# MeryylleA/Lunaris-Orion

Hardware: AMD Instinct MI355X
Metric: 128x128 sprites/sec, VAE training step (train_hybrid.py _process_batch), latent_dim=512 (higher is better)
Workload: dtype f16; 1 GPU; VAE-only training step (fwd+MSE/KL+bwd+clip+AdamW), per-GPU batch 64, latent_dim 512, teacher scalar 0 (--reward_scale 0 --quality_weight 0; the full hybrid step of BASELINE config 3 is the config3_full_hybrid object of a --full run at N=1), gradient_accumulation_steps 1, fp16 MFMA operands / fp32 accumulate, fp32 master weights; global_batch=64, latent_dim=512, parallelism=single, linear_weight_gradients=factored (never materialised)

## Files before the change

lunaris_orion_amd/csrc/lo_wgrad2.hip:

```cpp
#include "lo_conv.h"
#include "lo_conv_dev.h"

struct Wgrad2Args {
  const f16* a;
  const f16* f;
  float* slab;
  int B, Hc, Wc, Ca, Cf;
  int nsplit, chunks_per_split, nchunks;
  int packed_elems;
  int Cin;
  int wofs[4];
};

template <bool CONVT>
__global__ __launch_bounds__(512) void lo_wgrad_s2_mt(Wgrad2Args a) {
  constexpr int R = CONVT ? 4 : 3, NTAP = R * R;
  constexpr int TH = 4, TW = 8;
  constexpr int PH = 2 * TH + R - 1, PWH = 10;
  constexpr int PROWS = PH * 2 * PWH;
  constexpr int PQ = (PROWS + 7) / 8;
  static_assert(4 + PQ <= 32, "eight waves x four instructions per chunk");
  constexpr int A_BYTES = 32 * 128, P_BYTES = PQ * 1024;
  constexpr int STAGE = A_BYTES + P_BYTES;
  constexpr int NSTAGE = 3, D = 2;
  constexpr int NTW = (NTAP + 1) / 2;
  __shared__ __attribute__((aligned(1024))) unsigned char smem[NSTAGE * STAGE + 1024];

  const int tid = threadIdx.x, lane = tid & 63;
  const int wave = __builtin_amdgcn_readfirstlane(tid >> 6);
  const int wa = wave & 1, wf = (wave >> 1) & 1, wt = wave >> 2;
  const int tiles_f = (a.Cf + 63) >> 6, tiles = (a.Ca >> 6) * tiles_f;
  const int wid = lo_xcd_remap(blockIdx.x, gridDim.x);
  const int tile = wid % tiles, split = wid / tiles;
  const int a0 = (tile / tiles_f) * 64, f0 = (tile % tiles_f) * 64;
  const int q_begin = split * a.chunks_per_split;
  const int q_end = min(a.nchunks, q_begin + a.chunks_per_split);
  const int nq = q_end - q_begin;
  const int chunks_x = a.Wc / TW, chunks_img = chunks_x * (a.Hc / TH);
  const int Hf = 2 * a.Hc, Wf = 2 * a.Wc;
  const f16* zpage = reinterpret_cast<const f16*>(lo_zero_page);

  int s_kind[4], s_off[4], s_py[4], s_px[4];
  unsigned int s_lds[4];
#pragma unroll
  for (int j = 0; j < 4; ++j) {
    const int q = wave * 4 + j;
    const int row8 = lane >> 3, pos = lane & 7;
    if (q < 4) {
      const int arow = q * 8 + row8;
      s_kind[j] = 0;
      s_py[j] = arow / TW; s_px[j] = arow % TW;
      s_off[j] = (s_py[j] * a.Wc + s_px[j]) * a.Ca + a0 + ((((pos >> 1) ^ lo_tr_swz<128>(arow)) << 1) | (pos & 1)) * 8;
      s_lds[j] = (unsigned int)(q * 1024);
    } else if (q - 4 < PQ) {
      const int prow = (q - 4) * 8 + row8;
      const int py = prow / (2 * PWH), rem = prow - py * (2 * PWH), par = rem / PWH, hx = rem - par * PWH;
      const int px = 2 * hx + par;
      const int ch = f0 + ((((pos >> 1) ^ lo_tr_swz<128>(prow)) << 1) | (pos & 1)) * 8;
      const bool ok = prow < PROWS && px < 2 * TW + R - 1 && ch < a.Cf;
      s_kind[j] = ok ? 1 : 2;
      s_py[j] = py - 1; s_px[j] = px - 1;
      s_off[j] = ((py - 1) * Wf + (px - 1)) * a.Cf + ch;
      s_lds[j] = (unsigned int)(A_BYTES + (q - 4) * 1024);
    } else {
      s_kind[j] = 2; s_py[j] = s_px[j] = 0; s_off[j] = 0;
      s_lds[j] = (unsigned int)(NSTAGE * STAGE);
    }
  }
  int nx_q = q_begin;
  int nx_n = nx_q / chunks_img, nx_y, nx_x;
  {
    const int r = nx_q - nx_n * chunks_img;
    nx_y = (r / chunks_x) * TH;
    nx_x = (r % chunks_x) * TW;
  }
  const unsigned int smem_base = (unsigned int)(size_t)smem;
  auto issue = [&](int stage) __attribute__((always_inline)) {
    const bool live = nx_q < q_end;
    const int y0 = nx_y, x0 = nx_x;
    const size_t abase = ((size_t)(nx_n * a.Hc + y0) * a.Wc + x0) * a.Ca;
    const size_t fbase = ((size_t)(nx_n * Hf + 2 * y0) * Wf + 2 * x0) * a.Cf;
#pragma unroll
    for (int j = 0; j < 4; ++j) {
      const f16* src = zpage;
      if (live && s_kind[j] == 0) src = a.a + abase + s_off[j];
      if (live && s_kind[j] == 1) {
        const int fy = 2 * y0 + s_py[j], fx = 2 * x0 + s_px[j];
        if ((unsigned)fy < (unsigned)Hf && (unsigned)fx < (unsigned)Wf) src = a.f + (ptrdiff_t)fbase + s_off[j];
      }
      const unsigned int dst = s_lds[j] >= (unsigned int)(NSTAGE * STAGE) ? smem_base + s_lds[j] : smem_base + stage * STAGE + s_lds[j];
      lo_dma16(src, dst);
    }
    ++nx_q;
    nx_x += TW;
    if (nx_x >= a.Wc) { nx_x = 0; nx_y += TH; if (nx_y >= a.Hc) { nx_y = 0; ++nx_n; } }
  };

  const int q16 = lane >> 4, i16 = lane & 15;
  const int trow = 4 * q16 + (i16 >> 2);
  const int tsub = (i16 & 3) * 8;
  int aoff[2][2];
#pragma unroll
  for (int mi = 0; mi < 2; ++mi)
#pragma unroll
    for (int h = 0; h < 2; ++h) {
      const int Rr = trow + 16 * h, blk = wa * 2 + mi;
      aoff[mi][h] = Rr * 128 + ((blk ^ lo_tr_swz<128>(Rr)) * 32) + tsub;
    }
  int boff[NTW][2];
#pragma unroll
  for (int tt = 0; tt < NTW; ++tt)
#pragma unroll
    for (int h = 0; h < 2; ++h) {
      const int t = wt * NTW + tt;
      const int tq = t < NTAP ? t : 0;
      const int r = tq / R, s = tq % R;
      const int kk = trow + 16 * h, ky = kk / TW, kx = kk % TW;
      const int prow = ((2 * ky + r) * 2 + (s & 1)) * PWH + kx + (s >> 1);
      boff[tt][h] = A_BYTES + prow * 128 + (((wf * 2) ^ lo_tr_swz<128>(prow)) * 32) + tsub;
    }

  f32x4 acc[NTW][2][2];
#pragma unroll
  for (int tt = 0; tt < NTW; ++tt)
#pragma unroll
    for (int mi = 0; mi < 2; ++mi)
#pragma unroll
      for (int ni = 0; ni < 2; ++ni) acc[tt][mi][ni] = (f32x4){0.f, 0.f, 0.f, 0.f};

  auto tr = [&](const unsigned char* p) __attribute__((always_inline)) {
    return __builtin_amdgcn_ds_read_tr16_b64_v4f16((h16x4 __attribute__((address_space(3)))*)p);
  };
  auto frag = [&](const unsigned char* lo_p, const unsigned char* hi_p) __attribute__((always_inline)) {
    h16x4 lo = tr(lo_p), hi = tr(hi_p);
    return (f16x8){(f16)lo[0], (f16)lo[1], (f16)lo[2], (f16)lo[3], (f16)hi[0], (f16)hi[1], (f16)hi[2], (f16)hi[3]};
  };
  const bool f_live = f0 + wf * 32 < a.Cf;

  if (nq > 0) {
#pragma unroll
    for (int s = 0; s < D; ++s) issue(s);
    int rs = 0, ws = D % NSTAGE;
    for (int it = 0; it < nq; ++it) {
      LO_VMCNT(4 * (D - 1));
      __builtin_amdgcn_s_barrier();
      issue(ws);
      if (f_live) {
        const unsigned char* sbase = smem + rs * STAGE;
        f16x8 af[2];
#pragma unroll
        for (int mi = 0; mi < 2; ++mi) af[mi] = frag(sbase + aoff[mi][0], sbase + aoff[mi][1]);
#pragma unroll
        for (int tt = 0; tt < NTW; ++tt) {
          if (NTAP % 2 == 0 || tt + 1 < NTW || wt == 0) {
            f16x8 bf[2];
#pragma unroll
            for (int ni = 0; ni < 2; ++ni) bf[ni] = frag(sbase + (boff[tt][0] ^ (ni * 32)), sbase + (boff[tt][1] ^ (ni * 32)));
#pragma unroll
            for (int mi = 0; mi < 2; ++mi)
#pragma unroll
              for (int ni = 0; ni < 2; ++ni)
                acc[tt][mi][ni] = __builtin_amdgcn_mfma_f32_16x16x32_f16(af[mi], bf[ni], acc[tt][mi][ni], 0, 0, 0);
          }
        }
      }
      rs = (rs + 1 == NSTAGE) ? 0 : rs + 1;
      ws = (ws + 1 == NSTAGE) ? 0 : ws + 1;
    }
    LO_VMCNT(0);
  }
  if (!f_live) return;
  float* slab = a.slab + (size_t)split * a.packed_elems;
#pragma unroll
  for (int tt = 0; tt < NTW; ++tt) {
    const int t = wt * NTW + tt;
    if (t >= NTAP) continue;
    const int r = t / R, s = t % R;
#pragma unroll
    for (int mi = 0; mi < 2; ++mi)
#pragma unroll
      for (int ni = 0; ni < 2; ++ni) {
        const int cf = f0 + wf * 32 + ni * 16 + (lane & 15);
#pragma unroll
        for (int j = 0; j < 4; ++j) {
          const int ca = a0 + wa * 32 + mi * 16 + (lane >> 4) * 4 + j;
          size_t idx;
          if (CONVT) {
            const int p = ((r & 1) ? 0 : 2) + ((s & 1) ? 0 : 1), tp = (r >> 1) * 2 + (s >> 1);
            idx = (size_t)a.wofs[p] + (size_t)cf * (4 * a.Cin) + tp * a.Cin + ca;
          } else {
            idx = (size_t)ca * (9 * a.Cin) + t * a.Cin + cf;
          }
          if (cf < a.Cf) slab[idx] = acc[tt][mi][ni][j];
        }
      }
  }
}

int lo_wgrad2_run(const LoGeom& g, const LoWgradChoice& p, const f16* x, const f16* dy, float* slab, hipStream_t st) {
  LO_REQUIRE(p.kernel == LO_WK_WGRAD2, "lo_wgrad2_run: the plan names another weight-gradient kernel");
  const bool s2 = !p.convt;
  Wgrad2Args a;
  a.a = s2 ? dy : x; a.f = s2 ? x : dy; a.slab = slab;
  a.B = g.B; a.Hc = s2 ? g.Hout : g.Hin; a.Wc = s2 ? g.Wout : g.Win;
  a.Ca = s2 ? g.Cout : g.Cin; a.Cf = s2 ? g.Cin : g.Cout;
  a.nchunks = p.units; a.nsplit = p.nsplit; a.chunks_per_split = p.units_per_split;
  a.packed_elems = lo_geom_packed_elems(g);
  a.Cin = g.Cin;
  for (int q = 0; q < 4; ++q) a.wofs[q] = q < g.n_phase ? g.wofs[q] : 0;
  if (s2) hipLaunchKernelGGL((lo_wgrad_s2_mt<false>), p.grid, p.block, 0, st, a);
  else hipLaunchKernelGGL((lo_wgrad_s2_mt<true>), p.grid, p.block, 0, st, a);
  LO_LAUNCH_CHECK("wgrad_s2_mt");
  return LO_OK;
}
```

lunaris_orion_amd/csrc/lo_wgrad3.hip:

```cpp
#include "lo_conv.h"
#include "lo_conv_dev.h"

struct Wgrad3Args {
  const f16* x;
  const f16* dy;
  float* slab;
  int B, H, W, Cin, Cout;
  int nsplit, chunks_per_split, nchunks;
  int packed_elems;
#ifdef LO_STAMPS
  unsigned long long* stamps;
#endif
};
#ifdef LO_STAMPS
unsigned long long* g_lo_wgrad3_stamps = nullptr;
#define LO_T() __builtin_amdgcn_s_memtime()
#endif

template <int TH, int TW>
__global__ __launch_bounds__(512) void lo_wgrad3x3_mt(Wgrad3Args a) {
  static_assert(TH * TW == 32 && TW % 8 == 0, "a chunk is one 32-pixel K step");
  constexpr int PWP = TW + 2, PROWS = (TH + 2) * PWP;
  constexpr int PQ = (PROWS + 7) / 8;
  constexpr int PJ = (PQ + 3) / 4;
  constexpr int A_BYTES = 32 * 128;
  constexpr int P_BYTES = PQ * 1024;
  constexpr int STAGE = A_BYTES + P_BYTES;
  constexpr int NSTAGE = 4, D = 3;
  constexpr int XCHG_BYTES = 4 * 144 * 64 * 4;
  constexpr int LDS_BYTES = 2 * NSTAGE * STAGE > XCHG_BYTES ? 2 * NSTAGE * STAGE : XCHG_BYTES;
  __shared__ __attribute__((aligned(1024))) unsigned char smem_all[LDS_BYTES];

  const int tid = threadIdx.x, lane = tid & 63;
  const int wave8 = __builtin_amdgcn_readfirstlane(tid >> 6);
  const int grp = wave8 >> 2, wave = wave8 & 3;
  unsigned char* const smem = smem_all + grp * (NSTAGE * STAGE);
  const int wco = wave & 1, wci = wave >> 1;
  const int tiles_ci = a.Cin >> 6, tiles = (a.Cout >> 6) * tiles_ci;
  const int wid = lo_xcd_remap(blockIdx.x, gridDim.x);
  const int tile = wid % tiles, split = wid / tiles;
  const int co0 = (tile / tiles_ci) * 64, ci0 = (tile % tiles_ci) * 64;
  const int q_begin = split * a.chunks_per_split;
  const int q_end = min(a.nchunks, q_begin + a.chunks_per_split);
  const int nq = q_end - q_begin;
  const int chunks_x = a.W / TW, chunks_img = chunks_x * (a.H / TH);
  const f16* zpage = reinterpret_cast<const f16*>(lo_zero_page);

  const int drow = wave * 8 + (lane >> 3), dpos = lane & 7;
  const int d_ty = drow / TW, d_tx = drow % TW;
  const int d_lane = (d_ty * a.W + d_tx) * a.Cout + co0 + ((((dpos >> 1) ^ lo_tr_swz<128>(drow)) << 1) | (dpos & 1)) * 8;
  int p_py[PJ], p_px[PJ], p_lane[PJ];
#pragma unroll
  for (int j = 0; j < PJ; ++j) {
    const int prow = (j * 4 + wave) * 8 + (lane >> 3), pos = lane & 7;
    const int py = prow / PWP, px = prow - py * PWP;
    p_py[j] = prow < PROWS ? py - 1 : -100000;
    p_px[j] = px - 1;
    p_lane[j] = ((py - 1) * a.W + (px - 1)) * a.Cin + ci0 + ((((pos >> 1) ^ lo_tr_swz<128>(prow)) << 1) | (pos & 1)) * 8;
  }
  int nx_q = q_begin + grp;
  int nx_n = nx_q / chunks_img, nx_y, nx_x;
  {
    const int r = nx_q - nx_n * chunks_img;
    nx_y = (r / chunks_x) * TH;
    nx_x = (r % chunks_x) * TW;
  }
  auto issue = [&](int stage) __attribute__((always_inline)) {
    unsigned char* sa = smem + stage * STAGE;
    unsigned char* sp = sa + A_BYTES;
    const bool live = nx_q < q_end;
    const int y0 = nx_y, x0 = nx_x;
    const int pix0 = (nx_n * a.H + y0) * a.W + x0;
    {
      const f16* src = live ? a.dy + ((size_t)pix0 * a.Cout + d_lane) : zpage;
      lo_dma16(src, (unsigned int)(size_t)(sa + wave * 1024));
    }
#pragma unroll
    for (int j = 0; j < PJ; ++j) {
      if (j * 4 + wave < PQ) {
        const bool ok = live && (unsigned)(y0 + p_py[j]) < (unsigned)a.H && (unsigned)(x0 + p_px[j]) < (unsigned)a.W;
        const f16* src = ok ? a.x + ((size_t)pix0 * a.Cin + p_lane[j]) : zpage;
        lo_dma16(src, (unsigned int)(size_t)(sp + (j * 4 + wave) * 1024));
      }
    }
    nx_q += 2;
    nx_x += 2 * TW;
    if (nx_x >= a.W) {
      nx_x -= a.W; nx_y += TH;
      if (nx_x >= a.W) { nx_x -= a.W; nx_y += TH; }
      if (nx_y >= a.H) { nx_y -= a.H; ++nx_n; if (nx_y >= a.H) { nx_y -= a.H; ++nx_n; } }
    }
  };
  int lpt = 1;
#pragma unroll
  for (int j = 0; j < PJ; ++j) lpt += (j * 4 + wave < PQ) ? 1 : 0;

  const int q16 = lane >> 4, i16 = lane & 15;
  const int trow = 4 * q16 + (i16 >> 2);
  const int tsub = (i16 & 3) * 8;
  int aoff[2][2];
#pragma unroll
  for (int mi = 0; mi < 2; ++mi)
#pragma unroll
    for (int h = 0; h < 2; ++h) {
      const int R = trow + 16 * h, blk = wco * 2 + mi;
      aoff[mi][h] = R * 128 + ((blk ^ lo_tr_swz<128>(R)) * 32) + tsub;
    }
  int boff[9][2];
#pragma unroll
  for (int t = 0; t < 9; ++t)
#pragma unroll
    for (int h = 0; h < 2; ++h) {
      const int kk = trow + 16 * h;
      const int R = (kk / TW + t / 3) * PWP + kk % TW + t % 3;
      boff[t][h] = A_BYTES + R * 128 + (((wci * 2) ^ lo_tr_swz<128>(R)) * 32) + tsub;
    }

  f32x4 acc[9][2][2];
#pragma unroll
  for (int t = 0; t < 9; ++t)
#pragma unroll
    for (int mi = 0; mi < 2; ++mi)
#pragma unroll
      for (int ni = 0; ni < 2; ++ni) acc[t][mi][ni] = (f32x4){0.f, 0.f, 0.f, 0.f};

  auto tr = [&](const unsigned char* p) __attribute__((always_inline)) {
    return __builtin_amdgcn_ds_read_tr16_b64_v4f16((h16x4 __attribute__((address_space(3)))*)p);
  };
  auto frag = [&](const unsigned char* lo_p, const unsigned char* hi_p) __attribute__((always_inline)) {
    h16x4 lo = tr(lo_p), hi = tr(hi_p);
    return (f16x8){(f16)lo[0], (f16)lo[1], (f16)lo[2], (f16)lo[3], (f16)hi[0], (f16)hi[1], (f16)hi[2], (f16)hi[3]};
  };

  const int nit = (nq + 1) >> 1;
  auto compute = [&](int rs) __attribute__((always_inline)) {
    const unsigned char* sbase = smem + rs * STAGE;
    f16x8 af[2], bf[2][3][2];
#pragma unroll
    for (int mi = 0; mi < 2; ++mi) af[mi] = frag(sbase + aoff[mi][0], sbase + aoff[mi][1]);
#pragma unroll
    for (int tt = 0; tt < 3; ++tt)
#pragma unroll
      for (int ni = 0; ni < 2; ++ni) bf[0][tt][ni] = frag(sbase + (boff[tt][0] ^ (ni * 32)), sbase + (boff[tt][1] ^ (ni * 32)));
#pragma unroll
    for (int gq = 0; gq < 3; ++gq) {
      if (gq < 2) {
#pragma unroll
        for (int tt = 0; tt < 3; ++tt)
#pragma unroll
          for (int ni = 0; ni < 2; ++ni)
            bf[(gq + 1) & 1][tt][ni] = frag(sbase + (boff[3 * gq + 3 + tt][0] ^ (ni * 32)), sbase + (boff[3 * gq + 3 + tt][1] ^ (ni * 32)));
      }
#pragma unroll
      for (int tt = 0; tt < 3; ++tt)
#pragma unroll
        for (int mi = 0; mi < 2; ++mi)
#pragma unroll
          for (int ni = 0; ni < 2; ++ni)
            acc[3 * gq + tt][mi][ni] = __builtin_amdgcn_mfma_f32_16x16x32_f16(af[mi], bf[gq & 1][tt][ni], acc[3 * gq + tt][mi][ni], 0, 0, 0);
    }
  };
#ifdef LO_STAMPS
  const unsigned long long t_start = LO_T();
  unsigned long long t_loop = t_start, acc_w = 0, acc_i = 0, acc_c = 0;
#endif
  if (nit > 0) {
#pragma unroll
    for (int s = 0; s < D; ++s) issue(s);
#ifdef LO_STAMPS
    t_loop = LO_T();
#endif
    int rs = 0, ws = D % NSTAGE;
    for (int it = 0; it < nit; ++it) {
#ifdef LO_STAMPS
      const unsigned long long ta = LO_T();
#endif
      if (lpt == 4) LO_VMCNT(8); else if (lpt == 3) LO_VMCNT(6); else LO_VMCNT(4);
      __builtin_amdgcn_s_barrier();
#ifdef LO_STAMPS
      const unsigned long long tb = LO_T();
#endif
      if (grp == 0) issue(ws);
#ifdef LO_STAMPS
      const unsigned long long tc = LO_T();
#endif
      compute(rs);
#ifdef LO_STAMPS
      asm volatile("s_nop 0" ::: "memory");
      const unsigned long long td = LO_T();
#endif
      if (grp == 1) issue(ws);
#ifdef LO_STAMPS
      const unsigned long long te = LO_T();
      acc_w += tb - ta; acc_i += (tc - tb) + (te - td); acc_c += td - tc;
#endif
      rs = (rs + 1 == NSTAGE) ? 0 : rs + 1;
      ws = (ws + 1 == NSTAGE) ? 0 : ws + 1;
    }
    LO_VMCNT(0);
  }
#ifdef LO_STAMPS
  const unsigned long long t_loop_end = LO_T();
#endif
  __syncthreads();
  float* xch = reinterpret_cast<float*>(smem_all) + (size_t)wave * 144 * 64 + lane;
  if (grp == 1) {
#pragma unroll
    for (int t = 0; t < 9; ++t)
#pragma unroll
      for (int mi = 0; mi < 2; ++mi)
#pragma unroll
        for (int ni = 0; ni < 2; ++ni)
#pragma unroll
          for (int j = 0; j < 4; ++j) xch[(((t * 2 + mi) * 2 + ni) * 4 + j) * 64] = acc[t][mi][ni][j];
  }
  __syncthreads();
#ifdef LO_STAMPS
  if (a.stamps && lane == 0) {
    unsigned long long* d = a.stamps + ((size_t)blockIdx.x * 8 + wave8) * 16;
    d[0] = t_start; d[1] = t_loop; d[2] = t_loop_end; d[3] = LO_T(); d[4] = acc_w; d[5] = acc_i; d[6] = acc_c;
  }
#endif
  if (grp == 1) return;
#pragma unroll
  for (int t = 0; t < 9; ++t)
#pragma unroll
    for (int mi = 0; mi < 2; ++mi)
#pragma unroll
      for (int ni = 0; ni < 2; ++ni)
#pragma unroll
        for (int j = 0; j < 4; ++j) acc[t][mi][ni][j] += xch[(((t * 2 + mi) * 2 + ni) * 4 + j) * 64];
  float* slab = a.slab + (size_t)split * a.packed_elems;
  const int Ktot = 9 * a.Cin;
#pragma unroll
  for (int t = 0; t < 9; ++t)
#pragma unroll
    for (int mi = 0; mi < 2; ++mi)
#pragma unroll
      for (int ni = 0; ni < 2; ++ni) {
        const int c = ci0 + wci * 32 + ni * 16 + (lane & 15);
#pragma unroll
        for (int j = 0; j < 4; ++j) {
          const int n = co0 + wco * 32 + mi * 16 + (lane >> 4) * 4 + j;
          slab[(size_t)n * Ktot + t * a.Cin + c] = acc[t][mi][ni][j];
        }
      }
#ifdef LO_STAMPS
  if (a.stamps && lane == 0) a.stamps[((size_t)blockIdx.x * 8 + wave8) * 16 + 7] = LO_T();
#endif
}

int lo_wgrad3_run(const LoGeom& g, const LoWgradChoice& p, const f16* x, const f16* dy, float* slab, hipStream_t st) {
  LO_REQUIRE(p.kernel == LO_WK_WGRAD3, "lo_wgrad3_run: the plan names another weight-gradient kernel");
  Wgrad3Args a;
  a.x = x; a.dy = dy; a.slab = slab;
  a.B = g.B; a.H = g.Hin; a.W = g.Win; a.Cin = g.Cin; a.Cout = g.Cout;
  a.nchunks = p.units; a.nsplit = p.nsplit; a.chunks_per_split = p.units_per_split;
  a.packed_elems = lo_geom_packed_elems(g);
#ifdef LO_STAMPS
  a.stamps = g_lo_wgrad3_stamps;
#endif
  if (p.tw == 16) hipLaunchKernelGGL((lo_wgrad3x3_mt<2, 16>), p.grid, p.block, 0, st, a);
  else hipLaunchKernelGGL((lo_wgrad3x3_mt<4, 8>), p.grid, p.block, 0, st, a);
  LO_LAUNCH_CHECK("wgrad3x3_mt");
  return LO_OK;
}
```

Before: 23970 sprites/s.

## Repartition weight-gradient waves by tap groups with full 64-row A tiles

Both stride-2 and 3x3 weight-gradient kernels now give each wave all four 16-row A fragments and a subset of filter taps, instead of splitting A rows across waves and taps across fewer waves. Each A fragment read from LDS is reused across more MFMAs, and half-width Cf tiles now spread taps over all eight waves instead of idling half of them. In the stride-2 kernel the global DMA issue is split so that half the waves issue before computing and half after. In the 3x3 kernel the cross-group reduction exchange is rearranged by tap and folded directly into the slab store. The trade-off is more accumulator registers per wave (up to 5x4x2 f32x4), which raises register pressure and may reduce occupancy.

```diff
diff --git a/lunaris_orion_amd/csrc/lo_wgrad2.hip b/lunaris_orion_amd/csrc/lo_wgrad2.hip
--- a/lunaris_orion_amd/csrc/lo_wgrad2.hip
+++ b/lunaris_orion_amd/csrc/lo_wgrad2.hip
@@ -23,16 +23,19 @@
   constexpr int A_BYTES = 32 * 128, P_BYTES = PQ * 1024;
   constexpr int STAGE = A_BYTES + P_BYTES;
   constexpr int NSTAGE = 3, D = 2;
-  constexpr int NTW = (NTAP + 1) / 2;
+  constexpr int NTQ = (NTAP + 3) / 4;
   __shared__ __attribute__((aligned(1024))) unsigned char smem[NSTAGE * STAGE + 1024];
 
   const int tid = threadIdx.x, lane = tid & 63;
   const int wave = __builtin_amdgcn_readfirstlane(tid >> 6);
-  const int wa = wave & 1, wf = (wave >> 1) & 1, wt = wave >> 2;
   const int tiles_f = (a.Cf + 63) >> 6, tiles = (a.Ca >> 6) * tiles_f;
   const int wid = lo_xcd_remap(blockIdx.x, gridDim.x);
   const int tile = wid % tiles, split = wid / tiles;
   const int a0 = (tile / tiles_f) * 64, f0 = (tile % tiles_f) * 64;
+  const bool f_half = f0 + 32 >= a.Cf;
+  const int wf = f_half ? 0 : wave & 1, wt = f_half ? wave : wave >> 1;
+  const int t_each = f_half ? NTAP / 8 : NTAP / 4, t_rem = f_half ? NTAP % 8 : NTAP % 4;
+  const int t0 = wt * t_each + min(wt, t_rem), nt = t_each + (wt < t_rem ? 1 : 0);
   const int q_begin = split * a.chunks_per_split;
   const int q_end = min(a.nchunks, q_begin + a.chunks_per_split);
   const int nq = q_end - q_begin;
@@ -99,32 +102,31 @@
   const int q16 = lane >> 4, i16 = lane & 15;
   const int trow = 4 * q16 + (i16 >> 2);
   const int tsub = (i16 & 3) * 8;
-  int aoff[2][2];
-#pragma unroll
-  for (int mi = 0; mi < 2; ++mi)
+  int aoff[4][2];
+#pragma unroll
+  for (int mi = 0; mi < 4; ++mi)
 #pragma unroll
     for (int h = 0; h < 2; ++h) {
-      const int Rr = trow + 16 * h, blk = wa * 2 + mi;
-      aoff[mi][h] = Rr * 128 + ((blk ^ lo_tr_swz<128>(Rr)) * 32) + tsub;
-    }
-  int boff[NTW][2];
-#pragma unroll
-  for (int tt = 0; tt < NTW; ++tt)
+      const int Rr = trow + 16 * h;
+      aoff[mi][h] = Rr * 128 + ((mi ^ lo_tr_swz<128>(Rr)) * 32) + tsub;
+    }
+  int boff[NTQ][2];
+#pragma unroll
+  for (int tt = 0; tt < NTQ; ++tt)
 #pragma unroll
     for (int h = 0; h < 2; ++h) {
-      const int t = wt * NTW + tt;
-      const int tq = t < NTAP ? t : 0;
+      const int tq = tt < nt ? t0 + tt : 0;
       const int r = tq / R, s = tq % R;
       const int kk = trow + 16 * h, ky = kk / TW, kx = kk % TW;
       const int prow = ((2 * ky + r) * 2 + (s & 1)) * PWH + kx + (s >> 1);
       boff[tt][h] = A_BYTES + prow * 128 + (((wf * 2) ^ lo_tr_swz<128>(prow)) * 32) + tsub;
     }
 
-  f32x4 acc[NTW][2][2];
-#pragma unroll
-  for (int tt = 0; tt < NTW; ++tt)
-#pragma unroll
-    for (int mi = 0; mi < 2; ++mi)
+  f32x4 acc[NTQ][4][2];
+#pragma unroll
+  for (int tt = 0; tt < NTQ; ++tt)
+#pragma unroll
+    for (int mi = 0; mi < 4; ++mi)
 #pragma unroll
       for (int ni = 0; ni < 2; ++ni) acc[tt][mi][ni] = (f32x4){0.f, 0.f, 0.f, 0.f};
 
@@ -135,7 +137,6 @@
     h16x4 lo = tr(lo_p), hi = tr(hi_p);
     return (f16x8){(f16)lo[0], (f16)lo[1], (f16)lo[2], (f16)lo[3], (f16)hi[0], (f16)hi[1], (f16)hi[2], (f16)hi[3]};
   };
-  const bool f_live = f0 + wf * 32 < a.Cf;
 
   if (nq > 0) {
 #pragma unroll
@@ -144,46 +145,44 @@
     for (int it = 0; it < nq; ++it) {
       LO_VMCNT(4 * (D - 1));
       __builtin_amdgcn_s_barrier();
-      issue(ws);
-      if (f_live) {
-        const unsigned char* sbase = smem + rs * STAGE;
-        f16x8 af[2];
-#pragma unroll
-        for (int mi = 0; mi < 2; ++mi) af[mi] = frag(sbase + aoff[mi][0], sbase + aoff[mi][1]);
-#pragma unroll
-        for (int tt = 0; tt < NTW; ++tt) {
-          if (NTAP % 2 == 0 || tt + 1 < NTW || wt == 0) {
-            f16x8 bf[2];
-#pragma unroll
-            for (int ni = 0; ni < 2; ++ni) bf[ni] = frag(sbase + (boff[tt][0] ^ (ni * 32)), sbase + (boff[tt][1] ^ (ni * 32)));
-#pragma unroll
-            for (int mi = 0; mi < 2; ++mi)
-#pragma unroll
-              for (int ni = 0; ni < 2; ++ni)
-                acc[tt][mi][ni] = __builtin_amdgcn_mfma_f32_16x16x32_f16(af[mi], bf[ni], acc[tt][mi][ni], 0, 0, 0);
-          }
+      if (wave < 4) issue(ws);
+      const unsigned char* sbase = smem + rs * STAGE;
+      f16x8 af[4];
+#pragma unroll
+      for (int mi = 0; mi < 4; ++mi) af[mi] = frag(sbase + aoff[mi][0], sbase + aoff[mi][1]);
+#pragma unroll
+      for (int tt = 0; tt < NTQ; ++tt) {
+        if (tt < NTAP / 8 || tt < nt) {
+          f16x8 bf[2];
+#pragma unroll
+          for (int ni = 0; ni < 2; ++ni) bf[ni] = frag(sbase + (boff[tt][0] ^ (ni * 32)), sbase + (boff[tt][1] ^ (ni * 32)));
+#pragma unroll
+          for (int mi = 0; mi < 4; ++mi)
+#pragma unroll
+            for (int ni = 0; ni < 2; ++ni)
+              acc[tt][mi][ni] = __builtin_amdgcn_mfma_f32_16x16x32_f16(af[mi], bf[ni], acc[tt][mi][ni], 0, 0, 0);
         }
       }
+      if (wave >= 4) issue(ws);
       rs = (rs + 1 == NSTAGE) ? 0 : rs + 1;
       ws = (ws + 1 == NSTAGE) ? 0 : ws + 1;
     }
     LO_VMCNT(0);
   }
-  if (!f_live) return;
   float* slab = a.slab + (size_t)split * a.packed_elems;
 #pragma unroll
-  for (int tt = 0; tt < NTW; ++tt) {
-    const int t = wt * NTW + tt;
-    if (t >= NTAP) continue;
+  for (int tt = 0; tt < NTQ; ++tt) {
+    if (tt >= nt) continue;
+    const int t = t0 + tt;
     const int r = t / R, s = t % R;
 #pragma unroll
-    for (int mi = 0; mi < 2; ++mi)
+    for (int mi = 0; mi < 4; ++mi)
 #pragma unroll
       for (int ni = 0; ni < 2; ++ni) {
         const int cf = f0 + wf * 32 + ni * 16 + (lane & 15);
 #pragma unroll
         for (int j = 0; j < 4; ++j) {
-          const int ca = a0 + wa * 32 + mi * 16 + (lane >> 4) * 4 + j;
+          const int ca = a0 + mi * 16 + (lane >> 4) * 4 + j;
           size_t idx;
           if (CONVT) {
             const int p = ((r & 1) ? 0 : 2) + ((s & 1) ? 0 : 1), tp = (r >> 1) * 2 + (s >> 1);
diff --git a/lunaris_orion_amd/csrc/lo_wgrad3.hip b/lunaris_orion_amd/csrc/lo_wgrad3.hip
--- a/lunaris_orion_amd/csrc/lo_wgrad3.hip
+++ b/lunaris_orion_amd/csrc/lo_wgrad3.hip
@@ -27,7 +27,8 @@
   constexpr int P_BYTES = PQ * 1024;
   constexpr int STAGE = A_BYTES + P_BYTES;
   constexpr int NSTAGE = 4, D = 3;
-  constexpr int XCHG_BYTES = 4 * 144 * 64 * 4;
+  constexpr int NTW = 5;
+  constexpr int XCHG_BYTES = 2 * 9 * 32 * 64 * 4;
   constexpr int LDS_BYTES = 2 * NSTAGE * STAGE > XCHG_BYTES ? 2 * NSTAGE * STAGE : XCHG_BYTES;
   __shared__ __attribute__((aligned(1024))) unsigned char smem_all[LDS_BYTES];
 
@@ -35,7 +36,8 @@
   const int wave8 = __builtin_amdgcn_readfirstlane(tid >> 6);
   const int grp = wave8 >> 2, wave = wave8 & 3;
   unsigned char* const smem = smem_all + grp * (NSTAGE * STAGE);
-  const int wco = wave & 1, wci = wave >> 1;
+  const int wci = wave & 1, wt = (wave >> 1) ^ grp;
+  const int t0 = wt * NTW, nt = wt ? 9 - NTW : NTW;
   const int tiles_ci = a.Cin >> 6, tiles = (a.Cout >> 6) * tiles_ci;
   const int wid = lo_xcd_remap(blockIdx.x, gridDim.x);
   const int tile = wid % tiles, split = wid / tiles;
@@ -98,31 +100,32 @@
   const int q16 = lane >> 4, i16 = lane & 15;
   const int trow = 4 * q16 + (i16 >> 2);
   const int tsub = (i16 & 3) * 8;
-  int aoff[2][2];
-#pragma unroll
-  for (int mi = 0; mi < 2; ++mi)
+  int aoff[4][2];
+#pragma unroll
+  for (int mi = 0; mi < 4; ++mi)
 #pragma unroll
     for (int h = 0; h < 2; ++h) {
-      const int R = trow + 16 * h, blk = wco * 2 + mi;
-      aoff[mi][h] = R * 128 + ((blk ^ lo_tr_swz<128>(R)) * 32) + tsub;
-    }
-  int boff[9][2];
-#pragma unroll
-  for (int t = 0; t < 9; ++t)
+      const int R = trow + 16 * h;
+      aoff[mi][h] = R * 128 + ((mi ^ lo_tr_swz<128>(R)) * 32) + tsub;
+    }
+  int boff[NTW][2];
+#pragma unroll
+  for (int tt = 0; tt < NTW; ++tt)
 #pragma unroll
     for (int h = 0; h < 2; ++h) {
+      const int t = tt < nt ? t0 + tt : 0;
       const int kk = trow + 16 * h;
       const int R = (kk / TW + t / 3) * PWP + kk % TW + t % 3;
-      boff[t][h] = A_BYTES + R * 128 + (((wci * 2) ^ lo_tr_swz<128>(R)) * 32) + tsub;
-    }
-
-  f32x4 acc[9][2][2];
-#pragma unroll
-  for (int t = 0; t < 9; ++t)
-#pragma unroll
-    for (int mi = 0; mi < 2; ++mi)
-#pragma unroll
-      for (int ni = 0; ni < 2; ++ni) acc[t][mi][ni] = (f32x4){0.f, 0.f, 0.f, 0.f};
+      boff[tt][h] = A_BYTES + R * 128 + (((wci * 2) ^ lo_tr_swz<128>(R)) * 32) + tsub;
+    }
+
+  f32x4 acc[NTW][4][2];
+#pragma unroll
+  for (int tt = 0; tt < NTW; ++tt)
+#pragma unroll
+    for (int mi = 0; mi < 4; ++mi)
+#pragma unroll
+      for (int ni = 0; ni < 2; ++ni) acc[tt][mi][ni] = (f32x4){0.f, 0.f, 0.f, 0.f};
 
   auto tr = [&](const unsigned char* p) __attribute__((always_inline)) {
     return __builtin_amdgcn_ds_read_tr16_b64_v4f16((h16x4 __attribute__((address_space(3)))*)p);
@@ -135,29 +138,21 @@
   const int nit = (nq + 1) >> 1;
   auto compute = [&](int rs) __attribute__((always_inline)) {
     const unsigned char* sbase = smem + rs * STAGE;
-    f16x8 af[2], bf[2][3][2];
-#pragma unroll
-    for (int mi = 0; mi < 2; ++mi) af[mi] = frag(sbase + aoff[mi][0], sbase + aoff[mi][1]);
-#pragma unroll
-    for (int tt = 0; tt < 3; ++tt)
-#pragma unroll
-      for (int ni = 0; ni < 2; ++ni) bf[0][tt][ni] = frag(sbase + (boff[tt][0] ^ (ni * 32)), sbase + (boff[tt][1] ^ (ni * 32)));
-#pragma unroll
-    for (int gq = 0; gq < 3; ++gq) {
-      if (gq < 2) {
-#pragma unroll
-        for (int tt = 0; tt < 3; ++tt)
+    f16x8 af[4];
+#pragma unroll
+    for (int mi = 0; mi < 4; ++mi) af[mi] = frag(sbase + aoff[mi][0], sbase + aoff[mi][1]);
+#pragma unroll
+    for (int tt = 0; tt < NTW; ++tt) {
+      if (tt + 1 < NTW || nt == NTW) {
+        f16x8 bf[2];
+#pragma unroll
+        for (int ni = 0; ni < 2; ++ni) bf[ni] = frag(sbase + (boff[tt][0] ^ (ni * 32)), sbase + (boff[tt][1] ^ (ni * 32)));
+#pragma unroll
+        for (int mi = 0; mi < 4; ++mi)
 #pragma unroll
           for (int ni = 0; ni < 2; ++ni)
-            bf[(gq + 1) & 1][tt][ni] = frag(sbase + (boff[3 * gq + 3 + tt][0] ^ (ni * 32)), sbase + (boff[3 * gq + 3 + tt][1] ^ (ni * 32)));
+            acc[tt][mi][ni] = __builtin_amdgcn_mfma_f32_16x16x32_f16(af[mi], bf[ni], acc[tt][mi][ni], 0, 0, 0);
       }
-#pragma unroll
-      for (int tt = 0; tt < 3; ++tt)
-#pragma unroll
-        for (int mi = 0; mi < 2; ++mi)
-#pragma unroll
-          for (int ni = 0; ni < 2; ++ni)
-            acc[3 * gq + tt][mi][ni] = __builtin_amdgcn_mfma_f32_16x16x32_f16(af[mi], bf[gq & 1][tt][ni], acc[3 * gq + tt][mi][ni], 0, 0, 0);
     }
   };
 #ifdef LO_STAMPS
@@ -203,16 +198,18 @@
   const unsigned long long t_loop_end = LO_T();
 #endif
   __syncthreads();
-  float* xch = reinterpret_cast<float*>(smem_all) + (size_t)wave * 144 * 64 + lane;
+  float* xch = reinterpret_cast<float*>(smem_all) + (size_t)(wci * 9 + t0) * 32 * 64 + lane;
   if (grp == 1) {
 #pragma unroll
-    for (int t = 0; t < 9; ++t)
-#pragma unroll
-      for (int mi = 0; mi < 2; ++mi)
-#pragma unroll
-        for (int ni = 0; ni < 2; ++ni)
-#pragma unroll
-          for (int j = 0; j < 4; ++j) xch[(((t * 2 + mi) * 2 + ni) * 4 + j) * 64] = acc[t][mi][ni][j];
+    for (int tt = 0; tt < NTW; ++tt)
+      if (tt < nt) {
+#pragma unroll
+        for (int mi = 0; mi < 4; ++mi)
+#pragma unroll
+          for (int ni = 0; ni < 2; ++ni)
+#pragma unroll
+            for (int j = 0; j < 4; ++j) xch[(((tt * 4 + mi) * 2 + ni) * 4 + j) * 64] = acc[tt][mi][ni][j];
+      }
   }
   __syncthreads();
 #ifdef LO_STAMPS
@@ -222,29 +219,25 @@
   }
 #endif
   if (grp == 1) return;
-#pragma unroll
-  for (int t = 0; t < 9; ++t)
-#pragma unroll
-    for (int mi = 0; mi < 2; ++mi)
-#pragma unroll
-      for (int ni = 0; ni < 2; ++ni)
-#pragma unroll
-        for (int j = 0; j < 4; ++j) acc[t][mi][ni][j] += xch[(((t * 2 + mi) * 2 + ni) * 4 + j) * 64];
   float* slab = a.slab + (size_t)split * a.packed_elems;
   const int Ktot = 9 * a.Cin;
 #pragma unroll
-  for (int t = 0; t < 9; ++t)
-#pragma unroll
-    for (int mi = 0; mi < 2; ++mi)
-#pragma unroll
-      for (int ni = 0; ni < 2; ++ni) {
-        const int c = ci0 + wci * 32 + ni * 16 + (lane & 15);
-#pragma unroll
-        for (int j = 0; j < 4; ++j) {
-          const int n = co0 + wco * 32 + mi * 16 + (lane >> 4) * 4 + j;
-          slab[(size_t)n * Ktot + t * a.Cin + c] = acc[t][mi][ni][j];
+  for (int tt = 0; tt < NTW; ++tt) {
+    if (tt < nt) {
+#pragma unroll
+      for (int mi = 0; mi < 4; ++mi)
+#pragma unroll
+        for (int ni = 0; ni < 2; ++ni) {
+          const int c = ci0 + wci * 32 + ni * 16 + (lane & 15);
+#pragma unroll
+          for (int j = 0; j < 4; ++j) {
+            const int n = co0 + mi * 16 + (lane >> 4) * 4 + j;
+            slab[(size_t)n * Ktot + (t0 + tt) * a.Cin + c] = acc[tt][mi][ni][j] + xch[(((tt * 4 + mi) * 2 + ni) * 4 + j) * 64];
+          }
         }
-      }
+    }
+    __builtin_amdgcn_sched_barrier(0);
+  }
 #ifdef LO_STAMPS
   if (a.stamps && lane == 0) a.stamps[((size_t)blockIdx.x * 8 + wave8) * 16 + 7] = LO_T();
 #endif
```

Result: no change. 24150 sprites/s, median of 6 (+0.7%).
